# unanan/UNet_Nested4Tiny_Objects_Keypoints

Measured on AMD Instinct MI355X. Metric: images/sec (train step) UNet++ L=4 256x256, higher is better.
Workload: dtype f32

## Files before the change

### unet_nested4tiny_objects_keypoints_amd/csrc/gemm_wino.hip

```cpp
#include <cstdlib>
#include <utility>

#include "bn_fused.h"
#include "common.h"
#include "gemm_units.h"
#include "lds_asm.h"
#include "wino_experiments.h"

namespace unetpp {
namespace {

typedef float f32x2 __attribute__((ext_vector_type(2)));
typedef unsigned u32x4v __attribute__((vector_size(16)));
constexpr unsigned kOutOfRange = 0x80000000u;
typedef const __attribute__((address_space(1))) void* gptr_t;
typedef __attribute__((address_space(3))) void* lptr_t;

__device__ __forceinline__ void wino_input_transform(const float (&dd)[16], float (&V)[16]) {
  float t[4][4];
#pragma unroll
  for (int j = 0; j < 4; ++j) {
    t[0][j] = dd[0 + j] - dd[8 + j];
    t[1][j] = dd[4 + j] + dd[8 + j];
    t[2][j] = dd[8 + j] - dd[4 + j];
    t[3][j] = dd[4 + j] - dd[12 + j];
  }
#pragma unroll
  for (int i = 0; i < 4; ++i) {
    V[4 * i + 0] = t[i][0] - t[i][2];
    V[4 * i + 1] = t[i][1] + t[i][2];
    V[4 * i + 2] = t[i][2] - t[i][1];
    V[4 * i + 3] = t[i][1] - t[i][3];
  }
}

__device__ __forceinline__ void wino_input_transform_pk(const f32x2_t (&dd)[8], float (&V)[16]) {
  f32x2_t t[8];
#pragma unroll
  for (int p = 0; p < 2; ++p) {
    t[0 + p] = pk_sub(dd[0 + p], dd[4 + p]);
    t[2 + p] = pk_add(dd[2 + p], dd[4 + p]);
    t[4 + p] = pk_sub(dd[4 + p], dd[2 + p]);
    t[6 + p] = pk_sub(dd[2 + p], dd[6 + p]);
  }
#pragma unroll
  for (int i = 0; i < 4; ++i) {
    const f32x2_t va = pk_sub_add_x(t[2 * i], t[2 * i + 1]);
    const f32x2_t vb = pk_cross_sub(t[2 * i], t[2 * i + 1]);
    V[4 * i + 0] = va[0];
    V[4 * i + 1] = va[1];
    V[4 * i + 2] = vb[0];
    V[4 * i + 3] = vb[1];
  }
}

constexpr int WKC = 8;
constexpr int WNC = 32;
constexpr int WP = 10;
constexpr int WIMG = 4096;

#define WINO_FENCE() __builtin_amdgcn_sched_barrier(0)

template <int LOG2TW, int NH, int MODE, bool BNF = false>
__global__ __launch_bounds__(kThreads, 2) void gemm_wino_kernel(const FastArgs a) {
  constexpr bool LEAN = MODE != 0, FOLD = MODE == 2;
  constexpr int TW = 1 << LOG2TW, TH = kBlockPixels >> LOG2TW;
  constexpr int HWp = TW + 2, HHp = TH + 2;
  constexpr int NPIX = HWp * HHp;
  constexpr int TXN = TW / 2;
  constexpr int IN_FLOATS = 4096;
  constexpr int IN_ITEMS = (NPIX * 2 + kThreads - 1) / kThreads;
  constexpr int W_ITEMS = WIMG / 4 / kThreads;
  static_assert(IN_ITEMS == 3 && W_ITEMS == 4, "the staging lambdas' default ranges");
  static_assert(kMaxHaloPixels * WP <= IN_FLOATS, "input patch does not fit");
  static_assert(((IN_ITEMS * kThreads - 1) >> 1) * WP + 8 <= IN_FLOATS, "staging items past the patch must stay inside the buffer");
  constexpr int BUF = IN_FLOATS + WIMG;
  __shared__ __attribute__((aligned(16))) float smem[2 * BUF];
  float* in_tile = smem;
  float* w_tile = smem + IN_FLOATS;
  constexpr int RUN0 = 4 * WNC * 2;
  __shared__ float stat_lds[BNF ? RUN0 + kBnFusedMaxCols * 2 : RUN0];
  constexpr int kBiasCols = 512;
  __shared__ __attribute__((aligned(16))) float bias_lds[kBiasCols];

  const unetpp_gemm_desc& d = a.d;
  const int tid = threadIdx.x;
  const int wave = __builtin_amdgcn_readfirstlane(tid >> 6), lane = tid & 63, t16 = lane & 15, g = lane >> 4;

  const UnitRange ur = my_contiguous_unit_range(a.total_blocks);
  for (int i = tid; i < kBiasCols; i += kThreads)
    bias_lds[i] = (a.d.bias != nullptr && i < a.Ncols) ? a.d.bias[i] : 0.f;
  constexpr bool bn_fused = BNF;
  if constexpr (BNF) {
    for (int i = tid; i < kBnFusedMaxCols * 2; i += kThreads) stat_lds[RUN0 + i] = 0.f;
  }
  if (ur.count == 0) {
    if constexpr (BNF) {
      __syncthreads();
      bn_rows_store<kThreads>(a.d.stats_partial, a.Ncols, stat_lds + RUN0);
    }
    return;
  }
  const int n_units = __builtin_amdgcn_readfirstlane(static_cast<int>(ur.count));

  const int my_tile = 16 * wave + t16;
  const int a_base = ((2 * (my_tile / TXN)) * HWp + 2 * (my_tile % TXN)) * WP + 2 * g;
  const int b_base = (g * 16 + t16) * 2;

  f32x4 acc[16][NH];
#pragma unroll
  for (int xi = 0; xi < 16; ++xi)
#pragma unroll
    for (int nh = 0; nh < NH; ++nh) acc[xi][nh] = f32x4{0.f, 0.f, 0.f, 0.f};

  f32x4 reg_in[IN_ITEMS];
  unsigned voff[IN_ITEMS];
  unsigned in_mask = 0;
  int pf_cnt = 0;
  int p_unit = 0;
  int p_s = 0, p_c0 = 0, p_chunk = 0;
  int p_n = 0, p_ty0 = 0, p_tx0 = 0;
  const float* p_wimg = nullptr;
  const int cc = (tid & 1) << 2;
  const float* v_ptr = nullptr;
  const float* v_scale = nullptr;
  const float* v_shift = nullptr;
  int v_clen = 0;
  bool v_relu = false;
  int v_bytes = 0, v_pitch = 0, v_origin = 0;
  int pix[IN_ITEMS];
  auto cache_view = [&]() {
    const unetpp_view& V = d.in[p_s];
    v_clen = V.c_len;
    if constexpr (LEAN) {
      v_ptr = V.ptr;
      v_bytes = d.N * V.Hs * V.Ws * V.C * 4;
      v_pitch = V.C * 4;
      v_origin = V.c_off * 4;
      if constexpr (FOLD) {
        v_scale = V.scale;
        v_shift = V.shift;
        v_relu = V.relu != 0;
      }
    } else {
      v_ptr = V.ptr;
      v_scale = V.scale;
      v_shift = V.shift;
      v_relu = V.relu != 0;
    }
  };

  auto step_unit = [&](UnitGeom& u) {
    if (++u.group < a.n_groups) return;
    u.group = 0;
    ++u.patch;
    u.tx0 += TW;
    if (u.tx0 < a.tiles_x * TW) return;
    u.tx0 = 0;
    u.ty0 += TH;
    if (u.ty0 < a.tiles_y * TH) return;
    u.ty0 = 0;
    ++u.n;
  };
  UnitGeom p_ug = decode_unit<LOG2TW>(a, ur.first);
  p_ug.n = __builtin_amdgcn_readfirstlane(p_ug.n);
  p_ug.ty0 = __builtin_amdgcn_readfirstlane(p_ug.ty0);
  p_ug.tx0 = __builtin_amdgcn_readfirstlane(p_ug.tx0);
  p_ug.group = __builtin_amdgcn_readfirstlane(p_ug.group);
  p_ug.patch = __builtin_amdgcn_readfirstlane(static_cast<int>(p_ug.patch));
  UnitGeom c_ug = p_ug;

  long p_patch = -1;
  auto prefetch_unit = [&]() -> bool {
    const UnitGeom& ug = p_ug;
    p_wimg = d.weight_image + static_cast<long>(ug.group) * a.n_chunks * WIMG;
    if (ug.patch == p_patch) return true;
    p_patch = ug.patch;
    p_n = ug.n;
    p_ty0 = ug.ty0;
    p_tx0 = ug.tx0;
    if constexpr (LEAN) {
      const int row0 = p_n * d.H;
#pragma unroll
      for (int q = 0; q < IN_ITEMS; ++q) {
        const int it = tid + q * kThreads;
        const int hp = it >> 1;
        const int hy = hp / HWp, hx = hp - hy * HWp;
        const int y = p_ty0 + hy - 1, x = p_tx0 + hx - 1;
        const bool in_patch = ((q + 1) * kThreads <= NPIX * 2) ? true : (it < NPIX * 2);
        const bool inside = in_patch & (static_cast<unsigned>(y) < static_cast<unsigned>(d.H)) &
                            (static_cast<unsigned>(x) < static_cast<unsigned>(d.W));
        const int linear = (row0 + y) * d.W + x;
        pix[q] = inside ? linear : -1;
      }
      return false;
    }
    in_mask = 0;
#pragma unroll
    for (int q = 0; q < IN_ITEMS; ++q) {
      const int it = tid + q * kThreads;
      const int hp = it >> 1;
      const int hy = hp / HWp, hx = hp - hy * HWp;
      const int y = p_ty0 + hy - 1, x = p_tx0 + hx - 1;
      if ((it < NPIX * 2) && y >= 0 && y < d.H && x >= 0 && x < d.W) in_mask |= 1u << q;
    }
    return false;
  };
  auto view_offsets = [&](const unetpp_view& V) {
    if constexpr (LEAN) {
#pragma unroll
      for (int q = 0; q < IN_ITEMS; ++q)
        voff[q] = static_cast<unsigned>(pix[q] * v_pitch + v_origin + cc * 4) |
                  (static_cast<unsigned>(pix[q] >> 31) & kOutOfRange);
      return;
    }
#pragma unroll
    for (int q = 0; q < IN_ITEMS; ++q) {
      const int hp = min((tid + q * kThreads) >> 1, NPIX - 1);
      const int hy = hp / HWp, hx = hp - hy * HWp;
      const int yy = min(max(p_ty0 + hy - 1, 0), d.H - 1), xx = min(max(p_tx0 + hx - 1, 0), d.W - 1);
      voff[q] = view_pixel_offset32(V, p_n, yy, xx);
    }
  };
  auto advance = [&]() {
    if (p_chunk + 1 < a.n_chunks) {
      ++p_chunk;
      p_c0 += WKC;
      if (p_c0 >= v_clen) {
        ++p_s;
        p_c0 = 0;
        cache_view();
        view_offsets(d.in[p_s]);
      }
    } else if (p_unit + 1 < n_units) {
      ++p_unit;
      p_chunk = 0;
      p_c0 = 0;
      const bool same_view = p_s == 0;
      if (!same_view) {
        p_s = 0;
        cache_view();
      }
      step_unit(p_ug);
      if (!prefetch_unit() || !same_view) view_offsets(d.in[0]);
    }
  };
  f32x4 co_sc = {1.f, 1.f, 1.f, 1.f}, co_sh = {0.f, 0.f, 0.f, 0.f};
  float co_floor = 0.f;
  auto load_coeffs = [&]() {
    if constexpr (!FOLD) return;
    co_floor = v_relu ? 0.f : -__builtin_inff();
    if (v_scale != nullptr) {
      co_sc = *reinterpret_cast<const f32x4*>(v_scale + p_c0 + cc);
      co_sh = *reinterpret_cast<const f32x4*>(v_shift + p_c0 + cc);
    } else {
      co_sc = f32x4{1.f, 1.f, 1.f, 1.f};
      co_sh = f32x4{0.f, 0.f, 0.f, 0.f};
    }
  };
  auto load_inputs = [&]() {
    if constexpr (LEAN) {
      const __amdgpu_buffer_rsrc_t v_rsrc =
          __builtin_amdgcn_make_buffer_rsrc(const_cast<float*>(v_ptr), 0, v_bytes, 0x00020000);
#pragma unroll
      for (int q = 0; q < IN_ITEMS; ++q) {
        const u32x4v v = __builtin_amdgcn_raw_buffer_load_b128(v_rsrc, static_cast<int>(voff[q]), p_c0 * 4, 0);
        reg_in[q] = __builtin_bit_cast(f32x4, v);
      }
      return;
    }
    pf_cnt = min(WKC, v_clen - p_c0);
#pragma unroll
    for (int q = 0; q < IN_ITEMS; ++q) {
      const unsigned off = voff[q] + static_cast<unsigned>(p_c0 + (cc < pf_cnt ? cc : 0));
      reg_in[q] = *reinterpret_cast<const f32x4*>(v_ptr + off);
    }
  };
  auto dma_source = [&]() { return p_wimg + static_cast<long>(p_chunk) * WIMG; };
  auto dma_weights = [&](float* w_dst, const float* wp, int q0 = 0, int q1 = 4) {
#pragma unroll
    for (int q = q0; q < q1; ++q)
      __builtin_amdgcn_global_load_lds((gptr_t)(wp + (tid + q * kThreads) * 4),
                                       (lptr_t)(w_dst + (q * kThreads + wave * 64) * 4), 16, 0, 0);
  };
  auto store_chunk = [&](float* in_dst, int q0 = 0, int q1 = 3) {
    if constexpr (LEAN) {
#pragma unroll
      for (int q = q0; q < q1; ++q) {
        const int it = tid + q * kThreads;
        f32x4 v = reg_in[q];
        if constexpr (FOLD) {
          const unsigned inside = ~static_cast<unsigned>(pix[q] >> 31);
#pragma unroll
          for (int e = 0; e < 4; ++e)
            v[e] = __builtin_bit_cast(float, __builtin_bit_cast(unsigned, fmaxf(fmaf(v[e], co_sc[e], co_sh[e]), co_floor)) & inside);
        }
        *reinterpret_cast<f32x2*>(&in_dst[(it >> 1) * WP + cc]) = f32x2{v[0], v[1]};
        *reinterpret_cast<f32x2*>(&in_dst[(it >> 1) * WP + cc + 2]) = f32x2{v[2], v[3]};
      }
      return;
    }
    const bool affine = v_scale != nullptr;
    f32x4 sc = {1.f, 1.f, 1.f, 1.f}, sh = {0.f, 0.f, 0.f, 0.f};
    if (affine) {
      const int ch = p_c0 + (cc < pf_cnt ? cc : 0);
      sc = *reinterpret_cast<const f32x4*>(v_scale + ch);
      sh = *reinterpret_cast<const f32x4*>(v_shift + ch);
    }
#pragma unroll
    for (int q = 0; q < IN_ITEMS; ++q) {
      const int it = tid + q * kThreads;
      const bool keep = ((in_mask >> q) & 1u) && cc < pf_cnt;
      f32x4 v = reg_in[q];
      if (affine) {
#pragma unroll
        for (int e = 0; e < 4; ++e) v[e] = fmaf(v[e], sc[e], sh[e]);
      }
      if (v_relu) {
#pragma unroll
        for (int e = 0; e < 4; ++e) v[e] = fmaxf(v[e], 0.f);
      }
#pragma unroll
      for (int e = 0; e < 4; ++e) v[e] = keep ? v[e] : 0.f;
      if (it < NPIX * 2) {
        *reinterpret_cast<f32x2*>(&in_dst[(it >> 1) * WP + cc]) = f32x2{v[0], v[1]};
        *reinterpret_cast<f32x2*>(&in_dst[(it >> 1) * WP + cc + 2]) = f32x2{v[2], v[3]};
      }
    }
  };

  auto epilogue = [&]() {
    const UnitGeom& ug = c_ug;
    const TileCols tc = decode_tile(a, ug.group);
    const unetpp_view& O = d.out[tc.ov];
    const bool interior = (ug.ty0 + TH <= d.H) && (ug.tx0 + TW <= d.W);
    const unsigned rs = static_cast<unsigned>(O.sy) * O.Ws * O.C, cs = static_cast<unsigned>(O.sx) * O.C;
    const unsigned tile_base = view_pixel_offset32(O, ug.n, ug.ty0, ug.tx0) + tc.nt * WNC;
    float* obase = O.ptr + tile_base;
    const float* gbase = O.gate != nullptr ? O.gate + tile_base : nullptr;
    const bool vec_out = ((O.C | O.c_off | tc.n_cnt) & 3) == 0 && (reinterpret_cast<uintptr_t>(O.ptr) & 15) == 0 &&
                         (O.gate == nullptr || (reinterpret_cast<uintptr_t>(O.gate) & 15) == 0);
    const bool want_stats = d.stats_partial != nullptr;
    const float floor_v = O.relu ? 0.f : -__builtin_inff();
    float s1[NH][4], s2[NH][4];
#pragma unroll
    for (int nh = 0; nh < NH; ++nh)
#pragma unroll
      for (int rr = 0; rr < 4; ++rr) s1[nh][rr] = s2[nh][rr] = 0.f;
    if (d.bias != nullptr && tc.n0 + WNC <= kBiasCols) {
#pragma unroll
      for (int nh = 0; nh < NH; ++nh) acc[5][nh] += *reinterpret_cast<const f32x4*>(&bias_lds[tc.n0 + 16 * nh + 4 * g]);
    } else if (d.bias != nullptr) {
#pragma unroll
      for (int nh = 0; nh < NH; ++nh)
#pragma unroll
        for (int rr = 0; rr < 4; ++rr) {
          const int col = 16 * nh + 4 * g + rr;
          acc[5][nh][rr] += col < tc.n_cnt ? d.bias[tc.n0 + col] : 0.f;
        }
    }
    const unsigned ty2 = 2 * (my_tile / TXN), tx2 = 2 * (my_tile % TXN);
    auto out_row = [&](int ap, int nh, int rr, float (&y)[2]) {
      float tb[4];
#pragma unroll
      for (int b = 0; b < 4; ++b)
        tb[b] = (ap == 0) ? (acc[b][nh][rr] + acc[4 + b][nh][rr]) + acc[8 + b][nh][rr]
                          : (acc[4 + b][nh][rr] - acc[8 + b][nh][rr]) - acc[12 + b][nh][rr];
      y[0] = fmaxf((tb[0] + tb[1]) + tb[2], floor_v);
      y[1] = fmaxf((tb[1] - tb[2]) - tb[3], floor_v);
    };
    if (interior && vec_out && tc.n_cnt == 16 * NH) {
      const bool has_gate = gbase != nullptr, acc_out = O.accumulate != 0;
      const unsigned lane_off = ty2 * rs + tx2 * cs + 4 * g;
#pragma unroll
      for (int ap = 0; ap < 2; ++ap) {
        unsigned off[2][NH];
        f32x4 gt[2][NH], old[2][NH];
#pragma unroll
        for (int bp = 0; bp < 2; ++bp)
#pragma unroll
          for (int nh = 0; nh < NH; ++nh) off[bp][nh] = lane_off + ap * rs + bp * cs + 16 * nh;
        if (has_gate) {
#pragma unroll
          for (int bp = 0; bp < 2; ++bp)
#pragma unroll
            for (int nh = 0; nh < NH; ++nh) gt[bp][nh] = *reinterpret_cast<const f32x4*>(gbase + off[bp][nh]);
        }
        if (acc_out) {
#pragma unroll
          for (int bp = 0; bp < 2; ++bp)
#pragma unroll
            for (int nh = 0; nh < NH; ++nh) old[bp][nh] = *reinterpret_cast<const f32x4*>(obase + off[bp][nh]);
        }
        f32x4 yv[2][NH];
        const f32x2 floor2 = {floor_v, floor_v};
#pragma unroll
        for (int nh = 0; nh < NH; ++nh) {
          f32x2 y[2][2];
#pragma unroll
          for (int cp = 0; cp < 2; ++cp) {
            f32x2 tb[4];
#pragma unroll
            for (int b = 0; b < 4; ++b) {
              const f32x2 m0 = cp ? acc[b][nh].hi : acc[b][nh].lo, m1 = cp ? acc[4 + b][nh].hi : acc[4 + b][nh].lo;
              const f32x2 m2 = cp ? acc[8 + b][nh].hi : acc[8 + b][nh].lo, m3 = cp ? acc[12 + b][nh].hi : acc[12 + b][nh].lo;
              tb[b] = (ap == 0) ? (m0 + m1) + m2 : (m1 - m2) - m3;
            }
            y[0][cp] = __builtin_elementwise_max((tb[0] + tb[1]) + tb[2], floor2);
            y[1][cp] = __builtin_elementwise_max((tb[1] - tb[2]) - tb[3], floor2);
          }
          yv[0][nh] = f32x4{y[0][0].x, y[0][0].y, y[0][1].x, y[0][1].y};
          yv[1][nh] = f32x4{y[1][0].x, y[1][0].y, y[1][1].x, y[1][1].y};
          if (want_stats) {
#pragma unroll
            for (int rr = 0; rr < 4; ++rr) {
              const float y0 = yv[0][nh][rr], y1 = yv[1][nh][rr];
              s1[nh][rr] += y0 + y1;
              s2[nh][rr] = fmaf(y0, y0, fmaf(y1, y1, s2[nh][rr]));
            }
          }
        }
        if (!has_gate && !acc_out) {
#pragma unroll
          for (int bp = 0; bp < 2; ++bp)
#pragma unroll
            for (int nh = 0; nh < NH; ++nh) {
              if constexpr (wino_exp::kNoOutStore) asm volatile("" ::"v"(yv[bp][nh]), "v"(off[bp][nh]));
              else *reinterpret_cast<f32x4*>(obase + off[bp][nh]) = yv[bp][nh];
            }
          continue;
        }
#pragma unroll
        for (int bp = 0; bp < 2; ++bp)
#pragma unroll
          for (int nh = 0; nh < NH; ++nh) {
            f32x4 v = yv[bp][nh];
            if (has_gate && !O.gate_sum) {
#pragma unroll
              for (int e = 0; e < 4; ++e) v[e] = (gt[bp][nh][e] > 0.f) ? v[e] : 0.f;
            }
            if (acc_out) {
#pragma unroll
              for (int e = 0; e < 4; ++e) v[e] += old[bp][nh][e];
            }
            if (has_gate && O.gate_sum) {
#pragma unroll
              for (int e = 0; e < 4; ++e) v[e] = (gt[bp][nh][e] > 0.f) ? v[e] : 0.f;
            }
            *reinterpret_cast<f32x4*>(obase + off[bp][nh]) = v;
          }
      }
    } else {
#pragma unroll
      for (int ap = 0; ap < 2; ++ap) {
        const unsigned py = ty2 + ap;
#pragma unroll
        for (int nh = 0; nh < NH; ++nh)
#pragma unroll
          for (int rr = 0; rr < 4; ++rr) {
            float y[2];
            out_row(ap, nh, rr, y);
            const int col = 16 * nh + 4 * g + rr;
#pragma unroll
            for (int bp = 0; bp < 2; ++bp) {
              float v = y[bp];
              if ((col < tc.n_cnt) && (ug.ty0 + py < d.H) && (ug.tx0 + tx2 + bp < d.W)) {
                s1[nh][rr] += v;
                s2[nh][rr] = fmaf(v, v, s2[nh][rr]);
                const unsigned off = py * rs + (tx2 + bp) * cs + col;
                if (gbase != nullptr && !O.gate_sum) v = (gbase[off] > 0.f) ? v : 0.f;
                if (O.accumulate) v += obase[off];
                if (gbase != nullptr && O.gate_sum) v = (gbase[off] > 0.f) ? v : 0.f;
                obase[off] = v;
              }
            }
          }
      }
    }
#pragma unroll
    for (int xi = 0; xi < 16; ++xi)
#pragma unroll
      for (int nh = 0; nh < NH; ++nh) acc[xi][nh] = f32x4{0.f, 0.f, 0.f, 0.f};
    if (want_stats) {
#pragma unroll
      for (int nh = 0; nh < NH; ++nh)
#pragma unroll
        for (int rr = 0; rr < 4; ++rr) {
          s1[nh][rr] = row16_sum(s1[nh][rr]);
          s2[nh][rr] = row16_sum(s2[nh][rr]);
          if (t16 == 0) {
            stat_lds[(wave * WNC + 16 * nh + 4 * g + rr) * 2 + 0] = s1[nh][rr];
            stat_lds[(wave * WNC + 16 * nh + 4 * g + rr) * 2 + 1] = s2[nh][rr];
          }
        }
    }
  };
  auto flush_stats = [&]() {
    if (d.stats_partial == nullptr || tid >= 16 * NH) return;
    const UnitGeom& ug = c_ug;
    const TileCols tc = decode_tile(a, ug.group);
    if (tid >= tc.n_cnt) return;
    float t1 = 0.f, t2 = 0.f;
#pragma unroll
    for (int w = 0; w < 4; ++w) {
      t1 += stat_lds[(w * WNC + tid) * 2 + 0];
      t2 += stat_lds[(w * WNC + tid) * 2 + 1];
    }
    if constexpr (bn_fused) {
      stat_lds[RUN0 + (tc.n0 + tid) * 2 + 0] += t1;
      stat_lds[RUN0 + (tc.n0 + tid) * 2 + 1] += t2;
      return;
    }
    float* dst = d.stats_partial + (ug.patch * a.Ncols + tc.n0 + tid) * 2;
    dst[0] = t1;
    dst[1] = t2;
  };

  cache_view();
  prefetch_unit();
  view_offsets(d.in[0]);
  load_coeffs();
  load_inputs();
  dma_weights(w_tile, dma_source());
  store_chunk(in_tile);
  advance();
  load_coeffs();
  load_inputs();
  asm volatile("s_waitcnt vmcnt(%0)" ::"n"(IN_ITEMS) : "memory");
  __syncthreads();

  int c_chunk = 0, c_unit = 0;
  int cur = 0;
  while (true) {
    const unsigned in_b = lds_offset(in_tile) + a_base * 4, w_b = lds_offset(w_tile) + b_base * 4;
    float dd[16], ddn[16], V[16];
    f32x2_t dp[8], dpn[8];
    unsigned row_b[4];
#pragma unroll
    for (int i = 0; i < 4; ++i) row_b[i] = in_b + i * HWp * WP * 4;
    f32x4 us[2][2];
    if constexpr (LEAN) {
      static_for<8>([&](auto ic) {
        constexpr int e = decltype(ic)::v, j = 2 * (e & 1);
        lds_read2_b32<j * WP, (j + 1) * WP>(dp[e], row_b[e >> 1]);
      });
    } else {
      static_for<16>([&](auto ic) {
        constexpr int e = decltype(ic)::v;
        lds_read_b32<((e / 4) * HWp + (e % 4)) * WP * 4>(dd[e], in_b);
      });
    }
    lds_read2st64_b64<0, 1>(us[0][0], w_b);
    lds_read2st64_b64<2, 3>(us[0][1], w_b);

    float* other = smem + (cur ^ 1) * BUF;
    if constexpr (!LEAN) {
      __builtin_amdgcn_s_setprio(3);
      store_chunk(other);
      dma_weights(other + IN_FLOATS, dma_source());
      advance();
      load_inputs();
    }
    auto staging_piece = [&](auto gc) {
      constexpr int g = decltype(gc)::v;
      if constexpr (!LEAN) return;
      if constexpr (wino_exp::kNoStaging) {
        if constexpr (g == 2) advance();
        return;
      }
      if constexpr (g == 0 && !wino_exp::kNoStore) store_chunk(other);
      if constexpr (g == 0 && !wino_exp::kNoDma) dma_weights(other + IN_FLOATS, dma_source());
      if constexpr (g == 1) {
        advance();
        load_coeffs();
      }
      if constexpr (g == 2 && !wino_exp::kNoLoads) load_inputs();
    };

    __builtin_amdgcn_s_setprio(2);
    if constexpr (LEAN) {
      lds_wait8x2(dp);
      lds_wait(us[0][0], us[0][1]);
      wino_input_transform_pk(dp, V);
    } else {
      lds_wait16(dd);
      lds_wait(us[0][0], us[0][1]);
      wino_input_transform(dd, V);
    }
    static_for<8>([&](auto gc) {
      constexpr int g = decltype(gc)::v, cs = g & 1, ns = cs ^ 1;
      if constexpr (g + 1 < 8) {
        lds_read2st64_b64<4 * (g + 1), 4 * (g + 1) + 1>(us[ns][0], w_b);
        lds_read2st64_b64<4 * (g + 1) + 2, 4 * (g + 1) + 3>(us[ns][1], w_b);
      }
      if constexpr (g == 0) {
        if constexpr (LEAN) {
          static_for<8>([&](auto ic) {
            constexpr int e = decltype(ic)::v, j = 2 * (e & 1);
            lds_read2_b32<j * WP + 1, (j + 1) * WP + 1>(dpn[e], row_b[e >> 1]);
          });
        } else {
          static_for<16>([&](auto ic) {
            constexpr int e = decltype(ic)::v;
            lds_read_b32<(((e / 4) * HWp + (e % 4)) * WP + 1) * 4>(ddn[e], in_b);
          });
        }
      }
      WINO_FENCE();
#pragma unroll
      for (int q = 0; q < 4; ++q) {
        const int xi = (4 * g + q) & 15;
        const f32x4 up = us[cs][q >> 1];
        acc[xi][0] = __builtin_amdgcn_mfma_f32_16x16x4f32(up[(q & 1) * 2], V[xi], acc[xi][0], 0, 0, 0);
        if (NH == 2)
          acc[xi][NH - 1] = __builtin_amdgcn_mfma_f32_16x16x4f32(up[(q & 1) * 2 + 1], V[xi], acc[xi][NH - 1], 0, 0, 0);
      }
      staging_piece(gc);
      WINO_FENCE();
      if constexpr (g == 0) {
        if constexpr (LEAN) lds_wait8x2(dpn);
        else lds_wait16(ddn);
      }
      if constexpr (g + 1 < 8) lds_wait(us[ns][0], us[ns][1]);
      if constexpr (g == 3) {
        if constexpr (LEAN) wino_input_transform_pk(dpn, V);
        else wino_input_transform(ddn, V);
      }
    });
    __builtin_amdgcn_s_setprio(0);
    if constexpr (!wino_exp::kNoBarrier) {
      if (wino_exp::kLaxWait && c_chunk == 0 && c_unit > 0)
        asm volatile("s_waitcnt vmcnt(%0) lgkmcnt(0)" ::"n"(IN_ITEMS + 4 + 4 * NH) : "memory");
      else
      asm volatile("s_waitcnt vmcnt(%0) lgkmcnt(0)" ::"n"(IN_ITEMS) : "memory");
      __builtin_amdgcn_s_barrier();
      asm volatile("" ::: "memory");
    }
    if (c_chunk + 1 == a.n_chunks) {
#pragma unroll
      for (int q = 0; q < IN_ITEMS; ++q) asm volatile("" : "+v"(reg_in[q]));
      if constexpr (wino_exp::kNoEpilogue) {
#pragma unroll
        for (int xi = 0; xi < 16; ++xi)
#pragma unroll
          for (int nh = 0; nh < NH; ++nh) {
            asm volatile("" : "+v"(acc[xi][nh]));
            acc[xi][nh] = f32x4{0.f, 0.f, 0.f, 0.f};
          }
      } else {
        epilogue();
      }
      if (d.stats_partial != nullptr) {
        __syncthreads();
        flush_stats();
      }
      step_unit(c_ug);
      c_chunk = 0;
      if (++c_unit == n_units) break;
    } else {
      ++c_chunk;
    }
    cur ^= 1;
    in_tile = smem + cur * BUF;
    w_tile = in_tile + IN_FLOATS;
  }
  if constexpr (BNF) {
    __syncthreads();
    bn_rows_store<kThreads>(d.stats_partial, a.Ncols, stat_lds + RUN0);
  }
}

}

bool wino_applies(const unetpp_gemm_desc* d) {
  return d != nullptr && d->taps == 9 && (d->flags & (UNETPP_GEMM_DIRECT | UNETPP_GEMM_BF16)) == 0;
}

int launch_gemm_wino(const unetpp_gemm_desc* d, hipStream_t st, long* bn_rows) {
  FastArgs a;
  if (!wino_applies(d) || !fast_args(d, a, WKC, WNC) || d->weight_image == nullptr) return UNETPP_EINVAL;
  if (d->stats_partial != nullptr && d->n_out != 1) return UNETPP_EINVAL;
  const int cus = device_cu_count();
  if (cus <= 0) return UNETPP_ELAUNCH;
  long workers = (2L * cus) & ~7L;
#ifdef UNETPP_WINO_EXP
  if (opt_value(OPT_WINO_ONE_PER_CU, 0) == 1) workers = cus & ~7L;
#endif
  if (workers < 8) workers = 8;
  if (workers > kBnFusedRows) workers = kBnFusedRows;
  const dim3 grid(static_cast<unsigned>(a.total_blocks <= workers ? a.total_blocks : workers)), block(kThreads);
  bool narrow = true;
  for (int i = 0; i < d->n_out; ++i) narrow = narrow && d->out[i].c_len <= 16;
  bool lean = opt_value(OPT_WINO_NO_LEAN, 0) == 0, fold = false;
  for (int i = 0; i < d->n_in; ++i) {
    const unetpp_view& v = d->in[i];
    lean = lean && (v.c_len & 7) == 0 && v.Hs == d->H && v.Ws == d->W && v.sy == 1 && v.sx == 1 && v.oy == 0 &&
           v.ox == 0 && static_cast<long>(d->N) * v.Hs * v.Ws * v.C * 4 <= 0x7fffffffL;
    fold = fold || v.scale != nullptr || v.relu != 0;
  }
  const int mode = !lean ? 0 : (fold ? 2 : 1);
  a.bn_in_kernel = (mode != 0 && bn_rows_per_workgroup(d, a.Ncols)) ? 1 : 0;
#define UNETPP_LAUNCH_WINO_M(L, NHV)                                                                    \
  do {                                                                                                  \
    if (mode == 0) hipLaunchKernelGGL((gemm_wino_kernel<L, NHV, 0>), grid, block, 0, st, a);            \
    else if (a.bn_in_kernel && mode == 1) hipLaunchKernelGGL((gemm_wino_kernel<L, NHV, 1, true>), grid, block, 0, st, a); \
    else if (a.bn_in_kernel) hipLaunchKernelGGL((gemm_wino_kernel<L, NHV, 2, true>), grid, block, 0, st, a);             \
    else if (mode == 1) hipLaunchKernelGGL((gemm_wino_kernel<L, NHV, 1>), grid, block, 0, st, a);       \
    else hipLaunchKernelGGL((gemm_wino_kernel<L, NHV, 2>), grid, block, 0, st, a);                      \
  } while (0)
#define UNETPP_LAUNCH_WINO(L)                 \
  do {                                        \
    if (narrow) UNETPP_LAUNCH_WINO_M(L, 1);   \
    else UNETPP_LAUNCH_WINO_M(L, 2);          \
  } while (0)
  if (a.log2tw == 5) UNETPP_LAUNCH_WINO(5);
  else if (a.log2tw == 4) UNETPP_LAUNCH_WINO(4);
  else UNETPP_LAUNCH_WINO(3);
#undef UNETPP_LAUNCH_WINO
#undef UNETPP_LAUNCH_WINO_M
  note_kernel("gemm_wino_kernel");
  if (a.bn_in_kernel && bn_rows != nullptr) *bn_rows = grid.x;
  return launch_status();
}

}
```

Before: 1715.

## Trim Winograd GEMM kernel register state by reloading scalars from kernarg

Reworks the Winograd conv GEMM kernel's per-unit bookkeeping to lower register pressure. Counters now run down, the per-pixel index array is replaced by byte offsets built directly with 24-bit multiplies, and the weight source pointer advances by increment. View and coefficient parameters are re-read from the kernarg segment instead of being held in registers. When consecutive views share the same channel pitch, only the base pointer is rebased rather than recomputing all offsets. This adds scalar loads and more complex control flow, and adds a host-side guard limiting channel counts so the 24-bit multiply stays exact.

```diff
diff --git a/unet_nested4tiny_objects_keypoints_amd/csrc/gemm_wino.hip b/unet_nested4tiny_objects_keypoints_amd/csrc/gemm_wino.hip
--- a/unet_nested4tiny_objects_keypoints_amd/csrc/gemm_wino.hip
+++ b/unet_nested4tiny_objects_keypoints_amd/csrc/gemm_wino.hip
@@ -60,6 +60,11 @@
 constexpr int WIMG = 4096;
 
 #define WINO_FENCE() __builtin_amdgcn_sched_barrier(0)
+
+struct UnitPos {
+  int n, ty0, tx0;
+  int group;
+};
 
 template <int LOG2TW, int NH, int MODE, bool BNF = false>
 __global__ __launch_bounds__(kThreads, 2) void gemm_wino_kernel(const FastArgs a) {
@@ -76,8 +81,6 @@
   static_assert(((IN_ITEMS * kThreads - 1) >> 1) * WP + 8 <= IN_FLOATS, "staging items past the patch must stay inside the buffer");
   constexpr int BUF = IN_FLOATS + WIMG;
   __shared__ __attribute__((aligned(16))) float smem[2 * BUF];
-  float* in_tile = smem;
-  float* w_tile = smem + IN_FLOATS;
   constexpr int RUN0 = 4 * WNC * 2;
   __shared__ float stat_lds[BNF ? RUN0 + kBnFusedMaxCols * 2 : RUN0];
   constexpr int kBiasCols = 512;
@@ -117,31 +120,24 @@
   unsigned voff[IN_ITEMS];
   unsigned in_mask = 0;
   int pf_cnt = 0;
-  int p_unit = 0;
-  int p_s = 0, p_c0 = 0, p_chunk = 0;
-  int p_n = 0, p_ty0 = 0, p_tx0 = 0;
-  const float* p_wimg = nullptr;
+  int p_units_left = n_units - 1;
+  int p_chunks_left = a.n_chunks - 1;
+  int p_s = 0, p_c0 = 0;
+  const float* w_src = nullptr;
   const int cc = (tid & 1) << 2;
   const float* v_ptr = nullptr;
   const float* v_scale = nullptr;
   const float* v_shift = nullptr;
   int v_clen = 0;
   bool v_relu = false;
-  int v_bytes = 0, v_pitch = 0, v_origin = 0;
-  int pix[IN_ITEMS];
+  int v_bytes = 0;
+  int v_base = 0;
   auto cache_view = [&]() {
     const unetpp_view& V = d.in[p_s];
     v_clen = V.c_len;
     if constexpr (LEAN) {
       v_ptr = V.ptr;
       v_bytes = d.N * V.Hs * V.Ws * V.C * 4;
-      v_pitch = V.C * 4;
-      v_origin = V.c_off * 4;
-      if constexpr (FOLD) {
-        v_scale = V.scale;
-        v_shift = V.shift;
-        v_relu = V.relu != 0;
-      }
     } else {
       v_ptr = V.ptr;
       v_scale = V.scale;
@@ -150,109 +146,148 @@
     }
   };
 
-  auto step_unit = [&](UnitGeom& u) {
-    if (++u.group < a.n_groups) return;
+  typedef const __attribute__((address_space(4))) FastArgs* kargs_t;
+  auto kargs = [&]() {
+    kargs_t p = (kargs_t)__builtin_amdgcn_kernarg_segment_ptr();
+    asm volatile("" : "+s"(p));
+    return p;
+  };
+
+  auto in_block = [](int v) {
+    asm volatile("" : "+v"(v));
+    return v;
+  };
+
+  auto step_unit = [&](UnitPos& u) -> bool {
+    const kargs_t k = kargs();
+    if (++u.group < k->n_groups) return false;
     u.group = 0;
-    ++u.patch;
     u.tx0 += TW;
-    if (u.tx0 < a.tiles_x * TW) return;
+    if (u.tx0 < k->tiles_x * TW) return true;
     u.tx0 = 0;
     u.ty0 += TH;
-    if (u.ty0 < a.tiles_y * TH) return;
+    if (u.ty0 < k->tiles_y * TH) return true;
     u.ty0 = 0;
-    ++u.n;
-  };
-  UnitGeom p_ug = decode_unit<LOG2TW>(a, ur.first);
-  p_ug.n = __builtin_amdgcn_readfirstlane(p_ug.n);
-  p_ug.ty0 = __builtin_amdgcn_readfirstlane(p_ug.ty0);
-  p_ug.tx0 = __builtin_amdgcn_readfirstlane(p_ug.tx0);
-  p_ug.group = __builtin_amdgcn_readfirstlane(p_ug.group);
-  p_ug.patch = __builtin_amdgcn_readfirstlane(static_cast<int>(p_ug.patch));
-  UnitGeom c_ug = p_ug;
-
-  long p_patch = -1;
-  auto prefetch_unit = [&]() -> bool {
-    const UnitGeom& ug = p_ug;
-    p_wimg = d.weight_image + static_cast<long>(ug.group) * a.n_chunks * WIMG;
-    if (ug.patch == p_patch) return true;
-    p_patch = ug.patch;
-    p_n = ug.n;
-    p_ty0 = ug.ty0;
-    p_tx0 = ug.tx0;
-    if constexpr (LEAN) {
-      const int row0 = p_n * d.H;
-#pragma unroll
-      for (int q = 0; q < IN_ITEMS; ++q) {
-        const int it = tid + q * kThreads;
-        const int hp = it >> 1;
-        const int hy = hp / HWp, hx = hp - hy * HWp;
-        const int y = p_ty0 + hy - 1, x = p_tx0 + hx - 1;
-        const bool in_patch = ((q + 1) * kThreads <= NPIX * 2) ? true : (it < NPIX * 2);
-        const bool inside = in_patch & (static_cast<unsigned>(y) < static_cast<unsigned>(d.H)) &
-                            (static_cast<unsigned>(x) < static_cast<unsigned>(d.W));
-        const int linear = (row0 + y) * d.W + x;
-        pix[q] = inside ? linear : -1;
-      }
-      return false;
-    }
-    in_mask = 0;
+    u.n = __builtin_amdgcn_readfirstlane(u.n + 1);
+    return true;
+  };
+  UnitPos p_ug;
+  {
+    const UnitGeom ug = decode_unit<LOG2TW>(a, ur.first);
+    p_ug.n = __builtin_amdgcn_readfirstlane(ug.n);
+    p_ug.ty0 = __builtin_amdgcn_readfirstlane(ug.ty0);
+    p_ug.tx0 = __builtin_amdgcn_readfirstlane(ug.tx0);
+    p_ug.group = __builtin_amdgcn_readfirstlane(ug.group);
+  }
+  UnitPos c_ug = p_ug;
+  int c_patch = __builtin_amdgcn_readfirstlane(static_cast<int>(static_cast<unsigned>(ur.first) / static_cast<unsigned>(a.n_groups)));
+
+  auto patch_offsets = [&]() {
+    const kargs_t k = kargs();
+    const int p_n = p_ug.n, p_ty0 = p_ug.ty0, p_tx0 = p_ug.tx0;
+    const int H = k->d.H, W = k->d.W;
+    const int row0 = p_n * H;
+    const unsigned v_pitch = static_cast<unsigned>(k->d.in[p_s].C);
+    const unsigned v_origin = static_cast<unsigned>(k->d.in[p_s].c_off + cc);
 #pragma unroll
     for (int q = 0; q < IN_ITEMS; ++q) {
       const int it = tid + q * kThreads;
       const int hp = it >> 1;
       const int hy = hp / HWp, hx = hp - hy * HWp;
       const int y = p_ty0 + hy - 1, x = p_tx0 + hx - 1;
+      const bool in_patch = ((q + 1) * kThreads <= NPIX * 2) ? true : (it < NPIX * 2);
+      const bool inside = in_patch & (static_cast<unsigned>(y) < static_cast<unsigned>(H)) &
+                          (static_cast<unsigned>(x) < static_cast<unsigned>(W));
+      int linear = (row0 + y) * W;
+      asm("" : "+v"(linear));
+      const int pix = inside ? linear + x : -1;
+      const unsigned px = static_cast<unsigned>(pix);
+      const unsigned lo = __umul24(px & 0xfffu, v_pitch) + v_origin, hi = __umul24(px >> 12, v_pitch);
+      voff[q] = (((hi << 12) + lo) << 2) | (static_cast<unsigned>(pix >> 31) & kOutOfRange);
+    }
+  };
+  auto rebase_view = [&]() {
+    const kargs_t k = kargs();
+    if (k->d.in[p_s].C == k->d.in[v_base].C) {
+      v_ptr += k->d.in[p_s].c_off - k->d.in[v_base].c_off;
+    } else {
+      v_base = p_s;
+      patch_offsets();
+    }
+  };
+  auto prefetch_patch = [&]() {
+    const int p_ty0 = p_ug.ty0, p_tx0 = p_ug.tx0;
+    in_mask = 0;
+    const int te = in_block(tid);
+#pragma unroll
+    for (int q = 0; q < IN_ITEMS; ++q) {
+      const int it = te + q * kThreads;
+      const int hp = it >> 1;
+      const int hy = hp / HWp, hx = hp - hy * HWp;
+      const int y = p_ty0 + hy - 1, x = p_tx0 + hx - 1;
       if ((it < NPIX * 2) && y >= 0 && y < d.H && x >= 0 && x < d.W) in_mask |= 1u << q;
     }
-    return false;
   };
   auto view_offsets = [&](const unetpp_view& V) {
-    if constexpr (LEAN) {
-#pragma unroll
-      for (int q = 0; q < IN_ITEMS; ++q)
-        voff[q] = static_cast<unsigned>(pix[q] * v_pitch + v_origin + cc * 4) |
-                  (static_cast<unsigned>(pix[q] >> 31) & kOutOfRange);
-      return;
-    }
+    const int te = in_block(tid);
 #pragma unroll
     for (int q = 0; q < IN_ITEMS; ++q) {
-      const int hp = min((tid + q * kThreads) >> 1, NPIX - 1);
+      const int hp = min((te + q * kThreads) >> 1, NPIX - 1);
       const int hy = hp / HWp, hx = hp - hy * HWp;
-      const int yy = min(max(p_ty0 + hy - 1, 0), d.H - 1), xx = min(max(p_tx0 + hx - 1, 0), d.W - 1);
-      voff[q] = view_pixel_offset32(V, p_n, yy, xx);
+      const int yy = min(max(p_ug.ty0 + hy - 1, 0), d.H - 1), xx = min(max(p_ug.tx0 + hx - 1, 0), d.W - 1);
+      voff[q] = view_pixel_offset32(V, p_ug.n, yy, xx);
     }
   };
   auto advance = [&]() {
-    if (p_chunk + 1 < a.n_chunks) {
-      ++p_chunk;
+    if (p_chunks_left > 0) {
+      --p_chunks_left;
+      w_src += WIMG;
       p_c0 += WKC;
       if (p_c0 >= v_clen) {
         ++p_s;
         p_c0 = 0;
         cache_view();
-        view_offsets(d.in[p_s]);
-      }
-    } else if (p_unit + 1 < n_units) {
-      ++p_unit;
-      p_chunk = 0;
+        if constexpr (LEAN) rebase_view();
+        else view_offsets(d.in[p_s]);
+      }
+    } else if (p_units_left > 0) {
+      --p_units_left;
+      p_chunks_left = kargs()->n_chunks - 1;
       p_c0 = 0;
-      const bool same_view = p_s == 0;
-      if (!same_view) {
+      const int s_old = p_s;
+      if (s_old != 0) {
         p_s = 0;
         cache_view();
       }
-      step_unit(p_ug);
-      if (!prefetch_unit() || !same_view) view_offsets(d.in[0]);
+      if (step_unit(p_ug)) {
+        w_src = kargs()->d.weight_image;
+        if constexpr (LEAN) {
+          v_base = 0;
+          patch_offsets();
+        } else {
+          prefetch_patch();
+          view_offsets(d.in[0]);
+        }
+      } else {
+        w_src += WIMG;
+        if (s_old != 0) {
+          if constexpr (LEAN) rebase_view();
+          else view_offsets(d.in[0]);
+        }
+      }
     }
   };
   f32x4 co_sc = {1.f, 1.f, 1.f, 1.f}, co_sh = {0.f, 0.f, 0.f, 0.f};
   float co_floor = 0.f;
   auto load_coeffs = [&]() {
     if constexpr (!FOLD) return;
-    co_floor = v_relu ? 0.f : -__builtin_inff();
-    if (v_scale != nullptr) {
-      co_sc = *reinterpret_cast<const f32x4*>(v_scale + p_c0 + cc);
-      co_sh = *reinterpret_cast<const f32x4*>(v_shift + p_c0 + cc);
+    const kargs_t k = kargs();
+    const float* sc = k->d.in[p_s].scale;
+    const float* sh = k->d.in[p_s].shift;
+    co_floor = k->d.in[p_s].relu != 0 ? 0.f : -__builtin_inff();
+    if (sc != nullptr) {
+      co_sc = *reinterpret_cast<const f32x4*>(sc + p_c0 + cc);
+      co_sh = *reinterpret_cast<const f32x4*>(sh + p_c0 + cc);
     } else {
       co_sc = f32x4{1.f, 1.f, 1.f, 1.f};
       co_sh = f32x4{0.f, 0.f, 0.f, 0.f};
@@ -276,12 +311,16 @@
       reg_in[q] = *reinterpret_cast<const f32x4*>(v_ptr + off);
     }
   };
-  auto dma_source = [&]() { return p_wimg + static_cast<long>(p_chunk) * WIMG; };
-  auto dma_weights = [&](float* w_dst, const float* wp, int q0 = 0, int q1 = 4) {
-#pragma unroll
-    for (int q = q0; q < q1; ++q)
-      __builtin_amdgcn_global_load_lds((gptr_t)(wp + (tid + q * kThreads) * 4),
+  unsigned w_voff[W_ITEMS];
+#pragma unroll
+  for (int q = 0; q < W_ITEMS; ++q) w_voff[q] = (tid + q * kThreads) * 16;
+  auto dma_weights = [&](float* w_dst, int q0 = 0, int q1 = 4) {
+#pragma unroll
+    for (int q = q0; q < q1; ++q) {
+      asm volatile("" : "+v"(w_voff[q]));
+      __builtin_amdgcn_global_load_lds((gptr_t)(reinterpret_cast<const char*>(w_src) + w_voff[q]),
                                        (lptr_t)(w_dst + (q * kThreads + wave * 64) * 4), 16, 0, 0);
+    }
   };
   auto store_chunk = [&](float* in_dst, int q0 = 0, int q1 = 3) {
     if constexpr (LEAN) {
@@ -290,7 +329,7 @@
         const int it = tid + q * kThreads;
         f32x4 v = reg_in[q];
         if constexpr (FOLD) {
-          const unsigned inside = ~static_cast<unsigned>(pix[q] >> 31);
+          const unsigned inside = ~static_cast<unsigned>(static_cast<int>(voff[q]) >> 31);
 #pragma unroll
           for (int e = 0; e < 4; ++e)
             v[e] = __builtin_bit_cast(float, __builtin_bit_cast(unsigned, fmaxf(fmaf(v[e], co_sc[e], co_sh[e]), co_floor)) & inside);
@@ -330,7 +369,7 @@
   };
 
   auto epilogue = [&]() {
-    const UnitGeom& ug = c_ug;
+    const UnitPos& ug = c_ug;
     const TileCols tc = decode_tile(a, ug.group);
     const unetpp_view& O = d.out[tc.ov];
     const bool interior = (ug.ty0 + TH <= d.H) && (ug.tx0 + TW <= d.W);
@@ -497,8 +536,7 @@
   };
   auto flush_stats = [&]() {
     if (d.stats_partial == nullptr || tid >= 16 * NH) return;
-    const UnitGeom& ug = c_ug;
-    const TileCols tc = decode_tile(a, ug.group);
+    const TileCols tc = decode_tile(a, c_ug.group);
     if (tid >= tc.n_cnt) return;
     float t1 = 0.f, t2 = 0.f;
 #pragma unroll
@@ -511,27 +549,34 @@
       stat_lds[RUN0 + (tc.n0 + tid) * 2 + 1] += t2;
       return;
     }
-    float* dst = d.stats_partial + (ug.patch * a.Ncols + tc.n0 + tid) * 2;
+    float* dst = d.stats_partial + (static_cast<long>(c_patch) * a.Ncols + tc.n0 + tid) * 2;
     dst[0] = t1;
     dst[1] = t2;
   };
 
   cache_view();
-  prefetch_unit();
-  view_offsets(d.in[0]);
+  w_src = d.weight_image + static_cast<long>(p_ug.group) * a.n_chunks * WIMG;
+  if constexpr (LEAN) {
+    patch_offsets();
+  } else {
+    prefetch_patch();
+    view_offsets(d.in[0]);
+  }
   load_coeffs();
   load_inputs();
-  dma_weights(w_tile, dma_source());
-  store_chunk(in_tile);
+  dma_weights(smem + IN_FLOATS);
+  store_chunk(smem);
   advance();
   load_coeffs();
   load_inputs();
   asm volatile("s_waitcnt vmcnt(%0)" ::"n"(IN_ITEMS) : "memory");
   __syncthreads();
 
-  int c_chunk = 0, c_unit = 0;
+  int c_chunks_left = a.n_chunks, c_units_left = n_units;
   int cur = 0;
   while (true) {
+    const float* in_tile = smem + cur * BUF;
+    const float* w_tile = in_tile + IN_FLOATS;
     const unsigned in_b = lds_offset(in_tile) + a_base * 4, w_b = lds_offset(w_tile) + b_base * 4;
     float dd[16], ddn[16], V[16];
     f32x2_t dp[8], dpn[8];
@@ -557,7 +602,7 @@
     if constexpr (!LEAN) {
       __builtin_amdgcn_s_setprio(3);
       store_chunk(other);
-      dma_weights(other + IN_FLOATS, dma_source());
+      dma_weights(other + IN_FLOATS);
       advance();
       load_inputs();
     }
@@ -569,7 +614,7 @@
         return;
       }
       if constexpr (g == 0 && !wino_exp::kNoStore) store_chunk(other);
-      if constexpr (g == 0 && !wino_exp::kNoDma) dma_weights(other + IN_FLOATS, dma_source());
+      if constexpr (g == 0 && !wino_exp::kNoDma) dma_weights(other + IN_FLOATS);
       if constexpr (g == 1) {
         advance();
         load_coeffs();
@@ -629,14 +674,14 @@
     });
     __builtin_amdgcn_s_setprio(0);
     if constexpr (!wino_exp::kNoBarrier) {
-      if (wino_exp::kLaxWait && c_chunk == 0 && c_unit > 0)
+      if (wino_exp::kLaxWait && c_chunks_left == a.n_chunks && c_units_left < n_units)
         asm volatile("s_waitcnt vmcnt(%0) lgkmcnt(0)" ::"n"(IN_ITEMS + 4 + 4 * NH) : "memory");
       else
       asm volatile("s_waitcnt vmcnt(%0) lgkmcnt(0)" ::"n"(IN_ITEMS) : "memory");
       __builtin_amdgcn_s_barrier();
       asm volatile("" ::: "memory");
     }
-    if (c_chunk + 1 == a.n_chunks) {
+    if (--c_chunks_left == 0) {
 #pragma unroll
       for (int q = 0; q < IN_ITEMS; ++q) asm volatile("" : "+v"(reg_in[q]));
       if constexpr (wino_exp::kNoEpilogue) {
@@ -654,15 +699,11 @@
         __syncthreads();
         flush_stats();
       }
-      step_unit(c_ug);
-      c_chunk = 0;
-      if (++c_unit == n_units) break;
-    } else {
-      ++c_chunk;
+      if (--c_units_left == 0) break;
+      c_chunks_left = kargs()->n_chunks;
+      c_patch += step_unit(c_ug) ? 1 : 0;
     }
     cur ^= 1;
-    in_tile = smem + cur * BUF;
-    w_tile = in_tile + IN_FLOATS;
   }
   if constexpr (BNF) {
     __syncthreads();
@@ -695,7 +736,7 @@
   for (int i = 0; i < d->n_in; ++i) {
     const unetpp_view& v = d->in[i];
     lean = lean && (v.c_len & 7) == 0 && v.Hs == d->H && v.Ws == d->W && v.sy == 1 && v.sx == 1 && v.oy == 0 &&
-           v.ox == 0 && static_cast<long>(d->N) * v.Hs * v.Ws * v.C * 4 <= 0x7fffffffL;
+           v.ox == 0 && static_cast<long>(d->N) * v.Hs * v.Ws * v.C * 4 <= 0x7fffffffL && v.C < (1 << 24);
     fold = fold || v.scale != nullptr || v.relu != 0;
   }
   const int mode = !lean ? 0 : (fold ? 2 : 1);
```

Result: no change. 1718 (median of 3 runs) (+0.2%).
